# sachaMorin/dino

Measured on AMD Instinct MI355X. Metric: frames/sec (480x480, ViT-S/8) DINOSeg inference, higher is better.
Workload: dtype fp16 (linears, Q.K^T; P.V bf16; fp32 accumulate); 1 GPU; DINOSeg predict path: ViT-S/8 x12 blocks + MLP head, 480x480 uint8 frames, batch 32/GPU, frames resident in HBM; blocks=12, batch_per_gpu=32, global_batch=32, resolution=480, precision=fp16, streams=2, parallelism=dp1 (independent replicas, no data-path collective)

## Files before the change

dino_amd/csrc/kernels.h:

```cpp
#pragma once
#include <hip/hip_runtime.h>
#include <stdint.h>

struct dinoseg_augment_frame;

namespace dseg {

typedef uint16_t bf16_t;

enum GemmEpilogue {
    EPI_PLAIN = 0,
    EPI_RESID = 1,
    EPI_GELU = 2,
    EPI_RELU = 3,
    EPI_QKV = 4,
    EPI_PATCH = 5,
    EPI_BF16 = 6,
    EPI_ATOMIC = 7,
    EPI_DGELU = 8,
    EPI_DRELU = 9,
};

struct GemmParams {
    const bf16_t* A; long a_plane; int lda;
    const bf16_t* W; long w_plane;
    int M, N, K;
    int n_off;
    int n_valid;
    int dbg;
    int planes;
    int fmt;
    int epi;
    const float* bias;
    float* out_f32; int ldo_f32;
    bf16_t* out_bf16; long out_plane; int ldo;
    bf16_t* q; bf16_t* k; bf16_t* v; long qkv_plane;
    int ntok, npad, heads, dmodel; float qscale;
    const float* pos; int n_patches;
    const float* resid;
    bf16_t* aux_out;
    const bf16_t* aux_in; long aux_plane;
    int v_bf16;
    int dispatch_rows;
    int ksplit;
    long split_stride;
    const float* ln_x; float ln_eps;
};
int launch_gemm(const GemmParams& p, hipStream_t s);
int launch_gemm_small(const GemmParams& p, hipStream_t s);
bool gemm_big_supported(const GemmParams& p);
int launch_gemm_big(const GemmParams& p, hipStream_t s);

bool gemm_rs_supported(const GemmParams& p);
int launch_pack_rs(const float* W, int N, int K, int kind, bf16_t* dst, hipStream_t s, int fmt);
int launch_pack_rs_ln(const float* W, const float* gamma, const float* beta, const float* bias, int N, int K, bf16_t* dst_w, float* dst_bias,
                      hipStream_t s, int fmt);
int launch_gemm_rs(const GemmParams& p, hipStream_t s);

struct LnGemmParams {
    const float* X; int ldx;
    const float* gamma; const float* beta; float eps;
    const bf16_t* W; long w_plane;
    const float* bias;
    int M, N;
    int epi;
    bf16_t* out_bf16; long out_plane; int ldo;
    bf16_t* q; bf16_t* k; bf16_t* v; long qkv_plane; int ntok, npad, heads, dmodel; float qscale;
    bf16_t* a_out; long a_plane;
    bf16_t* aux_out; long aux_plane;
    int dbg;
    int fmt;
};
bool gemm_ln_supported(int K, int N, int planes, int epi, int dmodel);
long gemm_ln_slab_elems(int N, int K, int planes);
int launch_pack_slabs(const float* src, int N, int K, int planes, bf16_t* dst, hipStream_t s, int fmt = 0);
int launch_gemm_ln(const LnGemmParams& p, int K, int planes, hipStream_t s);

struct MlpFusedParams {
    float* X; int ldx;
    const float* gamma; const float* beta; float eps;
    const bf16_t* Wp;
    const float* b1; const float* b2;
    int M;
    int* queue;
    int n_long, sleep_max;
    const bf16_t* ctx;
    const bf16_t* Wproj;
    const float* bproj;
    const bf16_t* Wqkv;
    const float* bqkv; const float* gamma1; const float* beta1;
    bf16_t* q; bf16_t* k; bf16_t* v;
    int ntok, npad, heads; float qscale;
    int fmt;
};
long mlp_fused_qkv_pack_elems(int D);
int launch_pack_qkv(const float* W, int D, bf16_t* dst, hipStream_t s, int fmt = 0);
long mlp_fused_proj_pack_elems(int D);
int launch_pack_proj(const float* W, int D, bf16_t* dst, hipStream_t s, int fmt = 0);
bool mlp_fused_supported(int D, int F, int planes);
long mlp_fused_pack_elems(int D, int F);
int launch_pack_mlp(const float* W1, const float* W2, int D, int F, bf16_t* dst, hipStream_t s, int fmt = 0);
int launch_mlp_fused2(const MlpFusedParams& p, hipStream_t s);

struct MlpFused3Params {
    float* X;
    float eps;
    const bf16_t* Wp;
    const float* b2;
    int M;
    const bf16_t* ctx; long ctx_plane;
    const float* bproj;
    int fmt;
    bf16_t* q; bf16_t* k; bf16_t* v; long qkv_plane;
    int ntok, npad, heads; float qscale;
    int v_bf16;
};
struct MlpFused3Weights {
    const float* Wproj; const float* W1; const float* b1; const float* W2;
    const float* gamma2; const float* beta2;
    const float* Wqkv_next; const float* bqkv_next; const float* gamma1_next; const float* beta1_next;
};
bool mlp_fused3_supported(int D, int F, int planes);
long mlp_fused3_pack_elems(int D, int F);
int launch_pack_mlp3(const MlpFused3Weights& w, int D, int F, bf16_t* dst, hipStream_t s, int fmt);
int launch_mlp_fused3(const MlpFused3Params& p, hipStream_t s);
bool mlp_fused4_supported(int D, int F, int planes);
long mlp_fused4_pack_elems(int D, int F);
int launch_pack_mlp4(const MlpFused3Weights& w, int D, int F, bf16_t* dst, hipStream_t s, int fmt);
int launch_mlp_fused4(const MlpFused3Params& p, hipStream_t s);

struct Options {
    int gemm_ln = 1;
    int gemm_big = 1;
    int gemm_dbg = 0;
    int attn_dbg = 0;
    int mlp_fused = 1;
    int mlp_fused_min_rows = 12000;
    int mlp_fused3_min_rows = 10000;
    int mlp_stagger = 0;
    int mlp_grid = 0;
    int qkv_fused = 0;
    int mlp_fused4 = 0;
    int qkv_fused4 = 1;
    int qkv_fused3 = 1;
    int gemm_rs = 3;
    int gemm_rs_min_rows = 24000;
    int gemm_rs_ln = 1;
    int proj_fused = 1;
    int streams = 2;
    int split_min = 8;
    int route_ab = 0;
    int fp16_patch_planes = 1;
    int op_v_bf16 = 0;
    int op_fmt = 0;
    int deterministic = 0;
    int train_streams = 2;
    int splitk_tiles = 512;
    int attn_variant = 11 | 1024 | 65536;
};
Options& options();

struct AttnParams {
    const bf16_t* q; const bf16_t* k; const bf16_t* v; long qkv_plane;
    bf16_t* ctx; long ctx_plane;
    float* lse;
    int B, heads, ntok, npad, planes;
    int dbg;
    int shared_gpu;
// ... 169 lines not shown
```

dino_amd/csrc/mlp_fused2.hip:

```cpp
#include <stdio.h>

#include <vector>

#include "mlp_common.h"

namespace dseg {

namespace mf2 {
using namespace mfc;
constexpr int NP = 4, BM = NP * 32, THREADS = 2 * NP * 64;
constexpr int W1_OFF = 0, W2_OFF = 3 * W_TILE;
constexpr int P_OFF = W2_OFF + 2 * W_TILE;
constexpr int B1_OFF = P_OFF + NP * 2 * 2048;
constexpr int B2_OFF = B1_OFF + F * 4;
constexpr int G_OFF = B2_OFF + D * 4, BE_OFF = G_OFF + D * 4;
constexpr int BP_OFF = BE_OFF + D * 4;
constexpr int G1_OFF = BP_OFF + D * 4, BE1_OFF = G1_OFF + D * 4;
constexpr int BQ_OFF = BE1_OFF + D * 4;
constexpr int NQT = 3 * D / 32;
constexpr int LDS_BYTES = BQ_OFF + 3 * D * 4;
static_assert(LDS_BYTES <= 160 * 1024, "LDS budget");
constexpr int NPT = D / 32;
constexpr int CTX_OFF = W2_OFF, CTX_SLOT = BM * 64;
static_assert(6 * CTX_SLOT == 2 * W_TILE, "ctx ring = W2 ring");
constexpr int H_OFF = W2_OFF + W_TILE;
static_assert(H_OFF + NP * 8192 <= B1_OFF, "hand-off windows");
#ifndef MF2_RA
#define MF2_RA 4
#endif
constexpr int RA = MF2_RA, NFR = RA + 1;
}

#ifndef MF2_ABL
#define MF2_ABL 0
#endif

#ifndef MF2_NT
#define MF2_NT 0
#endif
template <class T>
__device__ __forceinline__ T mf2_ld(const T* p) {
    if (MF2_NT & 1) return __builtin_nontemporal_load(p);
    return *p;
}
template <class T>
__device__ __forceinline__ void mf2_st(T* p, const T& v) {
    if (MF2_NT & 2) __builtin_nontemporal_store(v, p);
    else *p = v;
}

#ifndef MF2_STAMP
#define MF2_STAMP 0
#endif
#define MF2_ST(role, item_k, idx)                                                                                         \
    do {                                                                                                                  \
        if (MF2_STAMP && (tid & 63) == 0 && (item_k) < 4) {                                                               \
            __builtin_amdgcn_sched_barrier(0);                                                                            \
            unsigned long long* d = reinterpret_cast<unsigned long long*>(p.queue) +                                      \
                                    ((((long)blockIdx.x * 2 + (role)) * 4 + (item_k)) * 16 + (idx)) * 2;                  \
            d[0] = __builtin_amdgcn_s_memrealtime();                                                                      \
            d[1] = __builtin_amdgcn_s_memtime();                                                                          \
            __builtin_amdgcn_sched_barrier(0);                                                                            \
        }                                                                                                                 \
    } while (0)

template <int FMT, class PieceFn>
__device__ __forceinline__ void mf2_proj_tile(f32x16 (&acc)[mfc::NDB], uint32_t a_w, uint32_t ap0, uint32_t ap1, PieceFn&& piece) {
    using namespace mf2;
    bf16x8 p0, p1, fr[NFR];
    mf_rd<0>(p0, ap0);
    mf_rd<0>(p1, ap1);
    auto issue_read = [&](auto g_tag) __attribute__((always_inline)) {
        constexpr int G = decltype(g_tag)::value;
        if constexpr (G < 12) mf_rd<(2 * G) * 1024>(fr[G % NFR], a_w);
        else mf_rd<(2 * (G - 12) + 1) * 1024>(fr[G % NFR], a_w);
    };
    mf_for(std::make_integer_sequence<int, RA>{}, issue_read);
    mf_for(std::make_integer_sequence<int, 24>{}, [&](auto g_tag) __attribute__((always_inline)) {
        constexpr int G = decltype(g_tag)::value;
        if constexpr (G + RA < 24) issue_read(std::integral_constant<int, G + RA>{});
        mf_wait<(23 - G < RA ? 23 - G : RA)>();
        acc[G % 12] = mfma32f<FMT>(fr[G % NFR], G < 12 ? p0 : p1, acc[G % 12]);
        __builtin_amdgcn_sched_barrier(0);
        if constexpr ((G & 1) == 0) piece(std::integral_constant<int, G / 2>{});
        __builtin_amdgcn_sched_barrier(0);
    });
}

template <bool PROJ, bool QKV, int FMT>
__global__ __launch_bounds__(mf2::THREADS, 2) void mlp_fused2_kernel(MlpFusedParams p) {
    static_assert(PROJ || !QKV, "the qkv tail needs the hand-off machinery of the projection build");
    using namespace mf2;
    extern __shared__ __attribute__((aligned(16))) char smem[];
    const int tid = threadIdx.x;
    const int wave = __builtin_amdgcn_readfirstlane(tid >> 6);
    const int pair = wave & 3;
    const bool is_b = wave >= 4;
    const int M = p.M;
    const int nitems = (M + BM - 1) / BM;
    if ((int)blockIdx.x >= nitems) return;

    {
        float* const sB1w = reinterpret_cast<float*>(smem + B1_OFF);
        for (int i = tid; i < F / 4; i += THREADS) reinterpret_cast<f32x4*>(sB1w)[i] = reinterpret_cast<const f32x4*>(p.b1)[i];
        for (int i = tid; i < 3 * D / 4; i += THREADS) {
            const int which = i / (D / 4), j = i - which * (D / 4);
            const float* src = which == 0 ? p.b2 : (which == 1 ? p.gamma : p.beta);
            if (PROJ && which == 0) src = p.bproj;
            reinterpret_cast<f32x4*>(smem + B2_OFF + which * D * 4)[j] = reinterpret_cast<const f32x4*>(src)[j];
        }
        if (PROJ)
            for (int i = tid; i < D / 4; i += THREADS) reinterpret_cast<f32x4*>(smem + BP_OFF)[i] = reinterpret_cast<const f32x4*>(p.b2)[i];
        if (QKV) {
            for (int i = tid; i < 2 * D / 4; i += THREADS)
                reinterpret_cast<f32x4*>(smem + G1_OFF)[i] = reinterpret_cast<const f32x4*>(i < D / 4 ? p.gamma1 : p.beta1)[i < D / 4 ? i : i - D / 4];
            for (int i = tid; i < 3 * D / 4; i += THREADS) reinterpret_cast<f32x4*>(smem + BQ_OFF)[i] = reinterpret_cast<const f32x4*>(p.bqkv)[i];
        }
    }
    if (p.sleep_max > 0 && (int)blockIdx.x >= p.n_long) {
        const int n_short = (int)gridDim.x - p.n_long;
        const int reps = (int)(((long)p.sleep_max * ((int)blockIdx.x - p.n_long + 1)) / n_short);
        for (int i = 0; i < reps; ++i) __builtin_amdgcn_s_sleep(127);
    }
    const uint32_t lds_base = (uint32_t)(size_t)(__attribute__((address_space(3))) char*)smem;
    const float* const sB1 = reinterpret_cast<const float*>(smem + B1_OFF);
    const float* const sB2 = reinterpret_cast<const float*>(smem + B2_OFF);
    const float* const sG = reinterpret_cast<const float*>(smem + G_OFF);
    const float* const sBe = reinterpret_cast<const float*>(smem + BE_OFF);
    auto uniform64 = [](uint64_t v) __attribute__((always_inline)) -> uint64_t {
        return (uint64_t)(uint32_t)__builtin_amdgcn_readfirstlane((uint32_t)v) |
               ((uint64_t)(uint32_t)__builtin_amdgcn_readfirstlane((uint32_t)(v >> 32)) << 32);
    };
// ... 79 lines not shown
            };
            if (item == (int)blockIdx.x) load_rows(xrow);
            if (wave == 4) MF2_ST(1, item_k, 1);

            auto step_b = [&](int s, auto kind_tag) __attribute__((always_inline)) {
                constexpr int KIND = decltype(kind_tag)::value;
                __builtin_amdgcn_s_barrier();
                const int v1 = s + 3;
                const bool has_w2 = PROJ ? (s >= 1 && s <= NT - 1) : s <= NT - 1, has_w1 = v1 != NT;
                const int t1 = v1 < NT ? v1 : v1 - (NT + 1);
                const bool nxt = PROJ && v1 > NT;
                uint64_t gsb[4];
                uint32_t gld[4];
                {
                    const uint32_t so2 = (uint32_t)s * TILE_BYTES + W_TILE + frag0;
                    const uint32_t so1 = (nxt ? (uint32_t)t1 * W_TILE : (uint32_t)t1 * TILE_BYTES) + frag0;
                    const uint32_t d2 = lds_base + W2_OFF + (uint32_t)(s & 1) * W_TILE + frag0;
                    const uint32_t d1 = lds_base + W1_OFF + (uint32_t)(t1 % 3) * W_TILE + frag0;
                    const uint64_t w1src = nxt ? (QKV ? wq : wpj) : wp;
                    gsb[0] = uniform64(wp + so2);
                    gsb[1] = uniform64(wp + so2 + 4096);
                    gsb[2] = uniform64(w1src + so1);
                    gsb[3] = uniform64(w1src + so1 + 4096);
                    gld[0] = __builtin_amdgcn_readfirstlane(d2);
                    gld[1] = __builtin_amdgcn_readfirstlane(d2 + 4096);
                    gld[2] = __builtin_amdgcn_readfirstlane(d1);
                    gld[3] = __builtin_amdgcn_readfirstlane(d1 + 4096);
                }
                const bool ctx_pre = PROJ && s == NT && item + (int)gridDim.x < nitems;
                uint32_t cvn[2] = {0u, 0u};
                if (ctx_pre) {
#pragma unroll
                    for (int j = 0; j < 2; ++j) {
                        const uint32_t rin = (uint32_t)(2 * pair + j) * 16 + (lane_i >> 2);
                        int rg = (item + (int)gridDim.x) * BM + (int)rin;
                        rg = rg < M ? rg : M - 1;
                        cvn[j] = (uint32_t)rg * (D * 2) + (((lane_i & 3) ^ ((rin >> 2) & 3)) << 4);
                    }
                }
                auto piece = [&](auto j_tag) __attribute__((always_inline)) {
                    constexpr int J = decltype(j_tag)::value;
                    if (MF2_ABL & 2) return;
                    if constexpr (PROJ && J < 6) {
                        if (ctx_pre) {
                            constexpr int T = J >> 1, JJ = J & 1;
                            mf_dma1<0>(cvn[JJ], uniform64(ctxb + T * 64),
                                       __builtin_amdgcn_readfirstlane(lds_base + CTX_OFF + T * CTX_SLOT + (uint32_t)(2 * pair + JJ) * 1024));
                        }
                    }
                    if (J < 6 ? !has_w2 : !has_w1) return;
                    constexpr int Q = J % 6, G4 = (J / 6) * 2 + (Q >= 4 ? 1 : 0), OFF = (Q & 3) * 1024;
                    mf_dma1<OFF>(lane16_i, gsb[G4], gld[G4]);
                };
                if constexpr (KIND == 0) {
                    mf_for(std::make_integer_sequence<int, 12>{}, piece);
                    asm volatile("s_waitcnt vmcnt(6)" ::: "memory");
                } else {
                    const uint32_t a2 = frag_rd_i + W2_OFF + (uint32_t)((s - 1) & 1) * W_TILE;
                    const uint32_t ap = p_rd_i + (uint32_t)((s - 1) & 1) * 2048;
                    bf16x8 p0, p1, fr[NFR];
                    mf_rd<0>(p0, ap);
                    mf_rd<1024>(p1, ap);
                    auto issue_read = [&](auto g_tag) __attribute__((always_inline)) {
                        constexpr int G = decltype(g_tag)::value;
                        if (MF2_ABL & 16) return;
                        if constexpr (G < 12) mf_rd<(2 * G) * 1024>(fr[G % NFR], a2);
                        else mf_rd<(2 * (G - 12) + 1) * 1024>(fr[G % NFR], a2);
                    };
                    mf_for(std::make_integer_sequence<int, RA>{}, issue_read);
                    mf_for(std::make_integer_sequence<int, 24>{}, [&](auto g_tag) __attribute__((always_inline)) {
                        constexpr int G = decltype(g_tag)::value;
                        if constexpr (G + RA < 24) issue_read(std::integral_constant<int, G + RA>{});
                        if (MF2_ABL & 16) fr[G % NFR] = p0;
                        else mf_wait<(23 - G < RA ? 23 - G : RA)>();
                        if (!(MF2_ABL & 8)) o[G % 12] = mfma32f<FMT>(fr[G % NFR], G < 12 ? p0 : p1, o[G % 12]);
                        __builtin_amdgcn_sched_barrier(0);
                        if constexpr ((G & 1) == 0) piece(std::integral_constant<int, G / 2>{});
                        __builtin_amdgcn_sched_barrier(0);
                    });
                    if (s == NT - 3) asm volatile("s_waitcnt vmcnt(0)" ::: "memory");
                    else asm volatile("s_waitcnt vmcnt(6)" ::: "memory");
                }
            };
            auto ln_handoff = [&](const float* sGam, const float* sBet) __attribute__((always_inline)) {
                float sum = 0.f;
#pragma unroll
                for (int db = 0; db < NDB; ++db)
#pragma unroll
                    for (int h = 0; h < 2; ++h)
                        sum += ((o[db][8 * h] + o[db][8 * h + 1]) + (o[db][8 * h + 2] + o[db][8 * h + 3])) +
                               ((o[db][8 * h + 4] + o[db][8 * h + 5]) + (o[db][8 * h + 6] + o[db][8 * h + 7]));
                sum += __shfl_xor(sum, 32);
                const float mean = sum * (1.0f / D);
                float qv = 0.f;
#pragma unroll
                for (int db = 0; db < NDB; ++db)
#pragma unroll
                    for (int q4 = 0; q4 < 4; ++q4) {
                        __builtin_amdgcn_sched_barrier(0);
                        float part = 0.f;
#pragma unroll
                        for (int e = 0; e < 4; ++e) {
                            const float dlt = o[db][4 * q4 + e] - mean;
                            part = fmaf(dlt, dlt, part);
                        }
                        qv += part;
                    }
                qv += __shfl_xor(qv, 32);
                const float rstd = 1.0f / sqrtf(qv * (1.0f / D) + p.eps);
                float mean_n = mean;
                asm volatile("" : "+v"(mean_n));
                char* const hw = smem + H_OFF + pair * 8192 + lane16_i;
#pragma unroll
                for (int r = 0; r < 3; ++r) {
                    if (r > 0) __builtin_amdgcn_s_barrier();
#pragma unroll
                    for (int kk = 0; kk < 8; ++kk) {
                        __builtin_amdgcn_sched_barrier(0);
                        const int k = r * 8 + kk;
                        const float* gp = sGam + k * 16 + lh_i * 8;
                        const float* bp = sBet + k * 16 + lh_i * 8;
                        const f32x4 g0 = *reinterpret_cast<const f32x4*>(gp), g1 = *reinterpret_cast<const f32x4*>(gp + 4);
                        const f32x4 e0 = *reinterpret_cast<const f32x4*>(bp), e1 = *reinterpret_cast<const f32x4*>(bp + 4);
                        float y[8];
#pragma unroll
                        for (int e = 0; e < 4; ++e) {
                            y[e] = (o[k >> 1][(k & 1) * 8 + e] - mean_n) * rstd * g0[e] + e0[e];
                            y[4 + e] = (o[k >> 1][(k & 1) * 8 + 4 + e] - mean_n) * rstd * g1[e] + e1[e];
                        }
                        uint4 u;
                        u.x = pack2<FMT>(y[0], y[1]);
                        u.y = pack2<FMT>(y[2], y[3]);
                        u.z = pack2<FMT>(y[4], y[5]);
                        u.w = pack2<FMT>(y[6], y[7]);
                        *reinterpret_cast<uint4*>(hw + kk * 1024) = u;
                    }
                    asm volatile("s_waitcnt lgkmcnt(0)" ::: "memory");
                    if (r < 2) __builtin_amdgcn_s_barrier();
                }
            };

            if constexpr (PROJ) {
                uint32_t cv[2];
#pragma unroll
                for (int j = 0; j < 2; ++j) {
                    const uint32_t rin = (uint32_t)(2 * pair + j) * 16 + (lane_i >> 2);
                    int rg = item * BM + (int)rin;
                    rg = rg < M ? rg : M - 1;
                    cv[j] = (uint32_t)rg * (D * 2) + (((lane_i & 3) ^ ((rin >> 2) & 3)) << 4);
                }
                const uint32_t cp0 = ctx_frag_addr(lr_i, lh_i);
#pragma unroll 1
                for (int kt = 0; kt < NPT; ++kt) {
                    __builtin_amdgcn_s_barrier();
                    const bool issue = kt >= 1 && kt + 2 < NPT;
                    const int t = kt + 2;
                    const uint32_t so = (uint32_t)t * W_TILE + frag0;
                    const uint32_t d = lds_base + W1_OFF + (uint32_t)(t % 3) * W_TILE + frag0;
                    const uint32_t dc = lds_base + CTX_OFF + (uint32_t)(t % 6) * CTX_SLOT + (uint32_t)(2 * pair) * 1024;
                    const uint64_t gb0 = uniform64(wpj + so), gb1 = uniform64(wpj + so + 4096), cb = uniform64(ctxb + (uint32_t)t * 64);
                    const uint32_t gl0 = __builtin_amdgcn_readfirstlane(d), gl1 = __builtin_amdgcn_readfirstlane(d + 4096);
                    const uint32_t cl0 = __builtin_amdgcn_readfirstlane(dc), cl1 = __builtin_amdgcn_readfirstlane(dc + 1024);
                    auto piece = [&](auto j_tag) __attribute__((always_inline)) {
                        constexpr int J = decltype(j_tag)::value;
                        if ((MF2_ABL & 2) || !issue) return;
                        if constexpr (J < 4) mf_dma1<J * 1024>(lane16_i, gb0, gl0);
                        else if constexpr (J < 6) mf_dma1<(J - 4) * 1024>(lane16_i, gb1, gl1);
                        else if constexpr (J == 6) mf_dma1<0>(cv[0], cb, cl0);
                        else if constexpr (J == 7) mf_dma1<0>(cv[1], cb, cl1);
                    };
                    const uint32_t cs = (uint32_t)(kt % 6) * CTX_SLOT;
                    mf2_proj_tile<FMT>(o, frag_rd_i + W1_OFF + (uint32_t)(kt % 3) * W_TILE, cp0 + cs, (cp0 ^ 32u) + cs, piece);
                    if (issue) asm volatile("s_waitcnt vmcnt(8)" ::: "memory");
                    else asm volatile("s_waitcnt vmcnt(0)" ::: "memory");
                }
                if (wave == 4) MF2_ST(1, item_k, 9);
                __builtin_amdgcn_s_barrier();
                if (!(MF2_ABL & 2)) {
#pragma unroll
                    for (int t = 0; t < 4; ++t) {
                        const uint64_t sb = uniform64(wp + (t < 3 ? (uint32_t)t * TILE_BYTES : (uint32_t)W_TILE) + frag0);
                        const uint32_t ld = __builtin_amdgcn_readfirstlane(lds_base + (t < 3 ? W1_OFF + t * W_TILE : W2_OFF) + frag0);
                        mf_dma4(lane16_i, sb, ld);
                        mf_dma1<0>(lane16_i, sb + 4096, ld + 4096);
                        mf_dma1<1024>(lane16_i, sb + 4096, ld + 4096);
                    }
                }
                ln_handoff(sG, sBe);
                asm volatile("s_waitcnt vmcnt(0)" ::: "memory");
                if (wave == 4) MF2_ST(1, item_k, 10);
                __builtin_amdgcn_s_barrier();
                if (wave == 4) MF2_ST(1, item_k, 11);
            }
            step_b(0, std::integral_constant<int, 0>{});
            if (wave == 4) MF2_ST(1, item_k, 2);
#pragma unroll 1
            for (int s = 1; s <= NT; ++s) {
                step_b(s, std::integral_constant<int, 1>{});
                if (wave == 4 && s == 1) MF2_ST(1, item_k, 3);
                if (wave == 4 && s == 24) MF2_ST(1, item_k, 4);
                if (wave == 4 && s == 47) MF2_ST(1, item_k, 5);
            }
            if (wave == 4) MF2_ST(1, item_k, 6);

            if constexpr (QKV) {
                const bool has_next = item + (int)gridDim.x < nitems;
                {
                    const float* fp = reinterpret_cast<const float*>(smem + BP_OFF) + lh_i * 8;
#pragma unroll
                    for (int k = 0; k < NKS; ++k) {
                        const f32x4 c0 = *reinterpret_cast<const f32x4*>(fp + k * 16), c1 = *reinterpret_cast<const f32x4*>(fp + k * 16 + 4);
#pragma unroll
                        for (int e = 0; e < 4; ++e) {
                            o[k >> 1][(k & 1) * 8 + e] += c0[e];
                            o[k >> 1][(k & 1) * 8 + 4 + e] += c1[e];
                        }
                    }
                }
                __builtin_amdgcn_s_barrier();
                ln_handoff(reinterpret_cast<const float*>(smem + G1_OFF), reinterpret_cast<const float*>(smem + BE1_OFF));
                asm volatile("s_waitcnt vmcnt(0)" ::: "memory");
                __builtin_amdgcn_s_barrier();
                const int fr_ = row_c / p.ntok, tok_ = row_c - fr_ * p.ntok;
                const long qkv_row = ((long)fr_ * p.heads * p.npad + tok_) * 64 + lh_i * 8;
                const float* const nxr = p.X + (long)((row + BM * (int)gridDim.x) < M ? row + BM * (int)gridDim.x : M - 1) * D + lh_i * 8;
                mf_for(std::make_integer_sequence<int, NQT + 1>{}, [&](auto t_tag) __attribute__((always_inline)) {
                    constexpr int T = decltype(t_tag)::value;
                    __builtin_amdgcn_s_barrier();
                    if constexpr (T >= 1) {
                        constexpr int TT = T - 1, WHICH = TT / NDB, HB = TT % NDB;
                        const char* pr = smem + P_OFF + pair * 4096 + lane16_i + (TT & 1) * 2048;
                        const uint4 u0 = *reinterpret_cast<const uint4*>(pr), u1 = *reinterpret_cast<const uint4*>(pr + 1024);
                        bf16_t* dst = (WHICH == 0 ? p.q : (WHICH == 1 ? p.k : p.v)) + qkv_row + (long)(HB >> 1) * p.npad * 64 + (HB & 1) * 32;
                        if (row < M) {
                            *reinterpret_cast<uint4*>(dst) = u0;
                            *reinterpret_cast<uint4*>(dst + 16) = u1;
                        }
                    }
                    if constexpr (T >= 1 && T <= NKS) {
                        constexpr int k = T - 1;
                        if (row < M) {
                            f32x4 a, b;
#pragma unroll
                            for (int e = 0; e < 4; ++e) {
                                a[e] = o[k >> 1][(k & 1) * 8 + e];
                                b[e] = o[k >> 1][(k & 1) * 8 + 4 + e];
                            }
                            mf2_st(reinterpret_cast<f32x4*>(xrow + k * 16), a);
                            mf2_st(reinterpret_cast<f32x4*>(xrow + k * 16 + 4), b);
                        }
                    }
                    if constexpr (T > NKS) {
                        if (has_next) {
                            load_rows_k(nxr, std::integral_constant<int, 2 * (T - NKS - 1)>{});
                            load_rows_k(nxr, std::integral_constant<int, 2 * (T - NKS - 1) + 1>{});
                        }
                    }
                });
                static_assert(NQT + 1 - NKS - 1 == NKS / 2, "row loads fill the steps behind the row stores");
                if (has_next && !(MF2_ABL & 2)) {
#pragma unroll
                    for (int t = 0; t < 3; ++t) {
                        const uint64_t sb = uniform64(wpj + (uint32_t)t * W_TILE + frag0);
                        const uint32_t ld = __builtin_amdgcn_readfirstlane(lds_base + W1_OFF + t * W_TILE + frag0);
                        mf_dma4(lane16_i, sb, ld);
                        mf_dma1<0>(lane16_i, sb + 4096, ld + 4096);
                        mf_dma1<1024>(lane16_i, sb + 4096, ld + 4096);
                    }
                }
                asm volatile("s_waitcnt vmcnt(0)" ::: "memory");
                continue;
            }
            if (MF2_ABL & 32) {
#pragma unroll
                for (int db = 0; db < NDB; ++db) asm volatile("" ::"v"(o[db]));
            } else if (row < M) {
#pragma unroll
                for (int k = 0; k < NKS; ++k) {
                    f32x4 a, b;
#pragma unroll
                    for (int e = 0; e < 4; ++e) {
                        a[e] = o[k >> 1][(k & 1) * 8 + e];
                        b[e] = o[k >> 1][(k & 1) * 8 + 4 + e];
                    }
                    if constexpr (PROJ) {
                        const float* fp = reinterpret_cast<const float*>(smem + BP_OFF) + k * 16 + lh_i * 8;
                        a += *reinterpret_cast<const f32x4*>(fp);
                        b += *reinterpret_cast<const f32x4*>(fp + 4);
                    }
                    mf2_st(reinterpret_cast<f32x4*>(xrow + k * 16), a);
                    mf2_st(reinterpret_cast<f32x4*>(xrow + k * 16 + 4), b);
                }
            }
            if (wave == 4) MF2_ST(1, item_k, 7);
            if (item + (int)gridDim.x < nitems) {
                const int nrow = row + BM * (int)gridDim.x;
                load_rows(p.X + (long)(nrow < M ? nrow : M - 1) * D + lh_i * 8);
            }
            if (wave == 4) MF2_ST(1, item_k, 8);
        }
        asm volatile("s_waitcnt vmcnt(0)" ::: "memory");
        return;
    }
// ... 70 lines not shown
        const int row = item * BM + pair * 32 + lr;
        const int row_c = row < M ? row : M - 1;
        const float* const xrow = p.X + (long)row_c * D + lh * 8;
        f32x4 x[2 * NKS];
#pragma unroll
        for (int k = 0; k < NKS; ++k) {
            if (MF2_ABL & 32) {
                x[2 * k] = f32x4{1.f, 2.f, (float)k, (float)lane_p};
                x[2 * k + 1] = x[2 * k];
            } else {
                x[2 * k] = mf2_ld(reinterpret_cast<const f32x4*>(xrow + k * 16));
                x[2 * k + 1] = mf2_ld(reinterpret_cast<const f32x4*>(xrow + k * 16 + 4));
            }
        }
        layernorm(x, lh);
        return s_zero(lane_p, sB1);
    };
#define MF2_GELU2 0
    constexpr int GELU_LAST = MF2_GELU2 ? 8 : 10;
    float ex[16], ea[16], eb[16], ec[16];
    uint32_t pd[8];
    auto gelu_op = [&](auto n_tag, auto i_tag, const f32x16& s) __attribute__((always_inline)) {
        constexpr int N = decltype(n_tag)::value, I = decltype(i_tag)::value;
        if constexpr (I == 0) ex[N] = s[N];
        if (MF2_ABL & 1) {
            if constexpr (I == GELU_LAST && (N & 1)) pd[N >> 1] = pack2<FMT>(ex[N - 1], ex[N]);
            return;
        }
        if constexpr (MF2_GELU2) {
            if constexpr (I == 1) eb[N] = ex[N] * ex[N];
            if constexpr (I == 2) ec[N] = fmaf(-1.00125610e-1f, eb[N], -2.30876530f);
            if constexpr (I == 3) ec[N] = ec[N] * ex[N];
            if constexpr (I == 4) ec[N] = __builtin_amdgcn_exp2f(ec[N]);
            if constexpr (I == 5) ec[N] = 1.0f + ec[N];
            if constexpr (I == 6) ec[N] = __builtin_amdgcn_rcpf(ec[N]);
            if constexpr (I == 7) ex[N] = ex[N] * ec[N];
        } else {
            if constexpr (I == 1) ea[N] = __builtin_amdgcn_fmed3f(ex[N], -8.0f, 8.0f);
            if constexpr (I == 2) eb[N] = ea[N] * ea[N];
            if constexpr (I == 3) ec[N] = fmaf(1.01537542e-3f, eb[N], -1.06782573e-1f);
            if constexpr (I == 4) ec[N] = fmaf(ec[N], eb[N], -2.30111381f);
            if constexpr (I == 5) ec[N] = ec[N] * ea[N];
            if constexpr (I == 6) ec[N] = __builtin_amdgcn_exp2f(ec[N]);
            if constexpr (I == 7) ec[N] = 1.0f + ec[N];
            if constexpr (I == 8) ec[N] = __builtin_amdgcn_rcpf(ec[N]);
            if constexpr (I == 9) ex[N] = ex[N] * ec[N];
        }
        if constexpr (I == GELU_LAST && (N & 1)) pd[N >> 1] = pack2<FMT>(ex[N - 1], ex[N]);
    };
    auto valu_slot = [&](auto g_tag, const f32x16& s) __attribute__((always_inline)) {
        constexpr int G = decltype(g_tag)::value;
        mf_for(std::make_integer_sequence<int, 16>{}, [&](auto n_tag) __attribute__((always_inline)) {
            constexpr int N = decltype(n_tag)::value;
            constexpr int SG = (14 * N) / 15;
            if constexpr (G >= SG && G - SG <= GELU_LAST) gelu_op(n_tag, std::integral_constant<int, G - SG>{}, s);
        });
    };

    if (wave == 0) MF2_ST(0, 0, 15);
    if constexpr (!PROJ) sa = prologue(blockIdx.x);
    int item_k = 0;
    for (int item = blockIdx.x; item < nitems; item += gridDim.x, ++item_k) {
        if (wave == 0) MF2_ST(0, item_k, 0);
        uint32_t zero = 0;
        asm volatile("" : "+v"(zero));
        const uint32_t lane_i = __builtin_amdgcn_mbcnt_hi(~0u, __builtin_amdgcn_mbcnt_lo(~0u, zero));
        const uint32_t lane16_i = lane_i * 16, lh_i = lane_i >> 5;
        const uint32_t frag_rd_i = lds_base + lane16_i;
        char* const p_wr = smem + P_OFF + pair * 4096 + lane16_i;
        const float* const b1_lane_p = sB1 + attn::sigma23((int)(lane_i & 31));
        constexpr uint32_t ONE = FMT == FMT_FP16 ? 0x3C00u : 0x3F80u;
        const uint4 ones_u = {lh_i == 0 ? (ONE << 16 | ONE) : 0u, lh_i == 0 ? ONE : 0u, 0u, 0u};
        auto receive_xn = [&]() __attribute__((always_inline)) {
            const char* const hr = smem + H_OFF + pair * 8192 + lane16_i;
#pragma unroll
            for (int r = 0; r < 3; ++r) {
                __builtin_amdgcn_s_barrier();
#pragma unroll
                for (int kk = 0; kk < 8; ++kk) xn[r * 8 + kk] = lds_frag(hr + kk * 1024);
                asm volatile("s_waitcnt lgkmcnt(0)" ::: "memory");
                if (r < 2) __builtin_amdgcn_s_barrier();
            }
        };
        if constexpr (PROJ) {
#pragma unroll 1
            for (int kt = 0; kt <= NPT; ++kt) __builtin_amdgcn_s_barrier();
            receive_xn();
            sa = s_zero((int)lane_i, sB1);
            if (wave == 0) MF2_ST(0, item_k, 10);
        }

        auto step_a = [&](f32x16& s_cur, f32x16& s_nxt, int s, auto last_tag) __attribute__((always_inline)) {
            constexpr bool LAST = decltype(last_tag)::value;
            bf16x8 bias_frag;
            if (!LAST) {
                const float bj = b1_lane_p[(s + 1) * HT];
                const uint32_t hi = pack2<FMT>(bj, 0.f);
                const float r1f = bj - lo_to_f32<FMT>(hi);
                const uint32_t mid = pack2<FMT>(r1f, 0.f);
                const uint32_t lo = pack2<FMT>(r1f - lo_to_f32<FMT>(mid), 0.f);
                const uint4 fu = {lh_i == 0 ? ((hi & 0xFFFFu) | (mid << 16)) : 0u, lh_i == 0 ? (lo & 0xFFFFu) : 0u, 0u, 0u};
                bias_frag = __builtin_bit_cast(bf16x8, fu);
            }
            __builtin_amdgcn_sched_barrier(0);
            __builtin_amdgcn_s_barrier();
            if constexpr (!LAST) {
                const uint32_t a1 = frag_rd_i + W1_OFF + (uint32_t)((s + 1) % 3) * W_TILE;
                bf16x8 fr[NFR];
                auto issue_read = [&](auto g_tag) __attribute__((always_inline)) {
                    constexpr int G = decltype(g_tag)::value;
                    if (MF2_ABL & 16) return;
                    mf_rd<G * 1024>(fr[G % NFR], a1);
                };
                mf_for(std::make_integer_sequence<int, RA>{}, issue_read);
                {
                    f32x16 z;
#pragma unroll
                    for (int r = 0; r < 16; ++r) z[r] = 0.f;
                    s_nxt = mfma32f<FMT>(bias_frag, __builtin_bit_cast(bf16x8, ones_u), z);
                }
                __builtin_amdgcn_sched_barrier(0);
                mf_for(std::make_integer_sequence<int, 24>{}, [&](auto g_tag) __attribute__((always_inline)) {
                    constexpr int G = decltype(g_tag)::value;
                    if constexpr (G + RA < 24) issue_read(std::integral_constant<int, G + RA>{});
                    if (MF2_ABL & 16) fr[G % NFR] = xn[(G + 1) % NKS];
                    else mf_wait<(23 - G < RA ? 23 - G : RA)>();
                    if (!(MF2_ABL & 4)) s_nxt = mfma32f<FMT>(fr[G % NFR], xn[G], s_nxt);
                    __builtin_amdgcn_sched_barrier(0);
                    valu_slot(g_tag, s_cur);
                    __builtin_amdgcn_sched_barrier(0);
                });
                valu_slot(std::integral_constant<int, 24>{}, s_cur);
            } else {
                mf_for(std::make_integer_sequence<int, 25>{}, [&](auto g_tag) __attribute__((always_inline)) { valu_slot(g_tag, s_cur); });
            }
            const uint4 u0 = {pd[0], pd[1], pd[2], pd[3]}, u1 = {pd[4], pd[5], pd[6], pd[7]};
            *reinterpret_cast<uint4*>(p_wr + (s & 1) * 2048) = u0;
            *reinterpret_cast<uint4*>(p_wr + (s & 1) * 2048 + 1024) = u1;
            asm volatile("s_waitcnt lgkmcnt(0)" ::: "memory");
            __builtin_amdgcn_sched_barrier(0);
        };
#pragma unroll 1
        for (int s = 0; s < NT - 2; s += 2) {
            step_a(sa, sb, s, std::false_type{});
            if (wave == 0 && s == 0) MF2_ST(0, item_k, 1);
            step_a(sb, sa, s + 1, std::false_type{});
            if (wave == 0 && s == 0) MF2_ST(0, item_k, 2);
            if (wave == 0 && s == 22) MF2_ST(0, item_k, 3);
        }
        if (wave == 0) MF2_ST(0, item_k, 4);
        step_a(sa, sb, NT - 2, std::false_type{});
        step_a(sb, sa, NT - 1, std::true_type{});
        if (wave == 0) MF2_ST(0, item_k, 5);
        __builtin_amdgcn_s_barrier();
        if (wave == 0) MF2_ST(0, item_k, 6);
        if constexpr (QKV) {
            __builtin_amdgcn_s_barrier();
            receive_xn();
            const float* const sBq = reinterpret_cast<const float*>(smem + BQ_OFF);
            const float* const bq_lane_p = sBq + attn::sigma23((int)(lane_i & 31));
            const uint32_t frag0 = (uint32_t)pair * 6 * 1024;
            sa = s_zero((int)lane_i, sBq);
            auto step_q = [&](f32x16& s_cur, f32x16& s_nxt, int t, auto last_tag) __attribute__((always_inline)) {
                constexpr bool LAST = decltype(last_tag)::value;
                bf16x8 bias_frag;
                if (!LAST) {
                    const float bj = bq_lane_p[(t + 1) * 32];
                    const uint32_t hi = pack2<FMT>(bj, 0.f);
                    const float r1f = bj - lo_to_f32<FMT>(hi);
                    const uint32_t mid = pack2<FMT>(r1f, 0.f);
                    const uint32_t lo = pack2<FMT>(r1f - lo_to_f32<FMT>(mid), 0.f);
// ... 114 lines not shown
    for (int idx = blockIdx.x * blockDim.x + threadIdx.x; idx < total; idx += gridDim.x * blockDim.x) {
        int t = idx;
        const int e = t & 7; t >>= 3;
        const int lane = t & 63; t >>= 6;
        const int frag = t % NKS, kt = t / NKS;
        const int i = attn::sigma23(lane & 31), h = lane >> 5, db = frag >> 1, s2 = frag & 1;
        dst[idx] = pack1(W[(long)(db * 32 + i) * D + kt * 32 + s2 * 16 + h * 8 + e], fmt);
    }
}
__global__ __launch_bounds__(256) void pack_qkv_kernel(const float* __restrict__ W, bf16_t* __restrict__ dst, int fmt) {
    using namespace mf2;
    const int total = NQT * NKS * 512;
    for (int idx = blockIdx.x * blockDim.x + threadIdx.x; idx < total; idx += gridDim.x * blockDim.x) {
        int t = idx;
        const int e = t & 7; t >>= 3;
        const int lane = t & 63; t >>= 6;
        const int frag = t % NKS, tile = t / NKS;
        const int i = attn::sigma23(lane & 31), h = lane >> 5;
        dst[idx] = pack1(W[(long)(tile * 32 + i) * D + frag * 16 + h * 8 + e], fmt);
    }
}
long mlp_fused_qkv_pack_elems(int Dm) { return Dm == mf2::D ? (long)mf2::NQT * mf2::W_TILE / 2 : 0; }
int launch_pack_qkv(const float* W, int Dm, bf16_t* dst, hipStream_t s, int fmt) {
    if (Dm != mf2::D) {
        dinoseg_set_error("pack_qkv: unsupported width %d", Dm);
        return -1;
    }
    hipLaunchKernelGGL(pack_qkv_kernel, dim3(432), dim3(256), 0, s, W, dst, fmt);
    DSEG_CHECK_HIP(hipGetLastError());
    return 0;
}

long mlp_fused_proj_pack_elems(int Dm) { return Dm == mf2::D ? (long)mf2::NPT * mf2::W_TILE / 2 : 0; }
int launch_pack_proj(const float* W, int Dm, bf16_t* dst, hipStream_t s, int fmt) {
    if (Dm != mf2::D) {
        dinoseg_set_error("pack_proj: unsupported width %d", Dm);
        return -1;
    }
    hipLaunchKernelGGL(pack_proj_kernel, dim3(144), dim3(256), 0, s, W, dst, fmt);
    DSEG_CHECK_HIP(hipGetLastError());
    return 0;
}

template <int FMT>
static int launch_mlp_fused2_fmt(const MlpFusedParams& p, hipStream_t s);

int launch_mlp_fused2(const MlpFusedParams& p, hipStream_t s) {
    return p.fmt == FMT_FP16 ? launch_mlp_fused2_fmt<FMT_FP16>(p, s) : launch_mlp_fused2_fmt<FMT_BF16>(p, s);
}

template <int FMT>
static int launch_mlp_fused2_fmt(const MlpFusedParams& p, hipStream_t s) {
    static PerDeviceOnce once;
    if (once.first()) {
        DSEG_CHECK_HIP(hipFuncSetAttribute(reinterpret_cast<const void*>(&mlp_fused2_kernel<false, false, FMT>),
                                           hipFuncAttributeMaxDynamicSharedMemorySize, mf2::LDS_BYTES));
        DSEG_CHECK_HIP(hipFuncSetAttribute(reinterpret_cast<const void*>(&mlp_fused2_kernel<true, false, FMT>),
                                           hipFuncAttributeMaxDynamicSharedMemorySize, mf2::LDS_BYTES));
        DSEG_CHECK_HIP(hipFuncSetAttribute(reinterpret_cast<const void*>(&mlp_fused2_kernel<true, true, FMT>),
                                           hipFuncAttributeMaxDynamicSharedMemorySize, mf2::LDS_BYTES));
        once.mark();
    }
    if (p.M <= 0 || p.ldx != mf2::D) {
        dinoseg_set_error("mlp_fused2: bad shape M=%d ldx=%d", p.M, p.ldx);
        return -1;
    }
    const int ncu = device_cu_count();
    if (ncu <= 0) return -2;
    const int nitems = (p.M + mf2::BM - 1) / mf2::BM;
    int grid;
    if (options().mlp_stagger > 0) {
        grid = nitems < ncu ? nitems : ncu;
    } else if (options().mlp_grid > 0) {
        grid = options().mlp_grid < ncu ? options().mlp_grid : ncu;
        if (grid > nitems) grid = nitems;
    } else {
        const int rounds = (nitems + ncu - 1) / ncu;
        grid = (nitems + rounds - 1) / rounds;
    }
    MlpFusedParams q = p;
    q.queue = nullptr;
    q.n_long = nitems % grid;
    q.sleep_max = q.n_long > 0 && nitems > grid ? options().mlp_stagger : 0;
#if MF2_STAMP
    static unsigned long long* sbuf = nullptr;
    const size_t sbytes = (size_t)grid * 2 * 4 * 16 * 2 * 8;
    if (!sbuf) DSEG_CHECK_HIP(hipMalloc(reinterpret_cast<void**>(&sbuf), 256 * 2 * 4 * 16 * 2 * 8));
    DSEG_CHECK_HIP(hipMemsetAsync(sbuf, 0, sbytes, s));
    q.queue = reinterpret_cast<int*>(sbuf);
#endif
    if (p.ctx) {
        if (!p.Wproj || !p.bproj) {
            dinoseg_set_error("mlp_fused2: ctx without the packed projection weight / bias");
            return -1;
        }
        if (p.Wqkv) {
            if (!p.bqkv || !p.gamma1 || !p.beta1 || !p.q || !p.k || !p.v || p.ntok <= 0 || p.npad < p.ntok || p.heads * 64 != mf2::D) {
                dinoseg_set_error("mlp_fused2: incomplete qkv tail (bias / norm1 / q / k / v / geometry)");
                return -1;
            }
            hipLaunchKernelGGL((mlp_fused2_kernel<true, true, FMT>), dim3(grid), dim3(mf2::THREADS), mf2::LDS_BYTES, s, q);
        } else {
            hipLaunchKernelGGL((mlp_fused2_kernel<true, false, FMT>), dim3(grid), dim3(mf2::THREADS), mf2::LDS_BYTES, s, q);
        }
    } else {
        if (p.Wqkv) {
            dinoseg_set_error("mlp_fused2: the qkv tail needs the projection in the same launch (ctx)");
            return -1;
        }
        hipLaunchKernelGGL((mlp_fused2_kernel<false, false, FMT>), dim3(grid), dim3(mf2::THREADS), mf2::LDS_BYTES, s, q);
    }
    DSEG_CHECK_HIP(hipGetLastError());
#if MF2_STAMP
    {
        static int calls = 0;
        if (++calls == 20) {
            DSEG_CHECK_HIP(hipStreamSynchronize(s));
            std::vector<unsigned long long> h(sbytes / 8);
            DSEG_CHECK_HIP(hipMemcpy(h.data(), sbuf, sbytes, hipMemcpyDeviceToHost));
            for (int role = 0; role < 2; ++role)
                for (int k = 0; k < 4; ++k) {
                    fprintf(stderr, "role %c item %d:", role ? 'B' : 'A', k);
                    for (int i = 0; i < 16; ++i) {
                        double sum = 0, sumc = 0;
                        int n = 0;
                        for (int b = 0; b < grid; ++b) {
                            const unsigned long long* d = &h[((((size_t)b * 2 + role) * 4 + k) * 16) * 2];
                            const unsigned long long* d0 = &h[((((size_t)b * 2 + 1) * 4 + 0) * 16) * 2];
                            if (d[2 * i] == 0 || d0[0] == 0) continue;
                            sum += (double)(d[2 * i] - d0[0]) * 0.01;
                            sumc += (double)(d[2 * i + 1] - d0[1]);
                            ++n;
                        }
                        if (n) fprintf(stderr, " [%d] %.1fus/%.0fkc", i, sum / n, sumc / n / 1e3);
                    }
                    fprintf(stderr, "\n");
                }
        }
    }
#endif
    return 0;
}

}
```

Baseline: 2603 frames/s.

## Swap projection DMA/MFMA roles between wave pairs and overlap first hidden step with LN handoff

Reassigns work inside the fused attention-projection/MLP kernel. The consumer-side waves now issue the projection weight and context DMAs, and the producer waves run the projection MFMAs directly from LDS without prefetching. The first MLP hidden-layer step is folded into receiving the normalized activations, so MFMA work starts while rounds arrive instead of after all three. The LN handoff also relaxes a vmcnt wait to let loads stay in flight. The old placement stays available through a flag, at the cost of extra code paths and a more delicate barrier/waitcnt protocol.

```diff
diff --git a/dino_amd/csrc/kernels.h b/dino_amd/csrc/kernels.h
--- a/dino_amd/csrc/kernels.h
+++ b/dino_amd/csrc/kernels.h
@@ -84,6 +84,7 @@
     int M;
     int* queue;
     int n_long, sleep_max;
+    int old_place;
     const bf16_t* ctx;
     const bf16_t* Wproj;
     const float* bproj;
diff --git a/dino_amd/csrc/mlp_fused2.hip b/dino_amd/csrc/mlp_fused2.hip
--- a/dino_amd/csrc/mlp_fused2.hip
+++ b/dino_amd/csrc/mlp_fused2.hip
@@ -48,6 +48,10 @@
     if (MF2_NT & 2) __builtin_nontemporal_store(v, p);
     else *p = v;
 }
+
+#ifndef MF2_PLACE
+#define MF2_PLACE 0
+#endif
 
 #ifndef MF2_STAMP
 #define MF2_STAMP 0
@@ -293,7 +297,7 @@
                     else asm volatile("s_waitcnt vmcnt(6)" ::: "memory");
                 }
             };
-            auto ln_handoff = [&](const float* sGam, const float* sBet) __attribute__((always_inline)) {
+            auto ln_handoff = [&](const float* sGam, const float* sBet, bool early) __attribute__((always_inline)) {
                 float sum = 0.f;
 #pragma unroll
                 for (int db = 0; db < NDB; ++db)
@@ -347,6 +351,7 @@
                         *reinterpret_cast<uint4*>(hw + kk * 1024) = u;
                     }
                     asm volatile("s_waitcnt lgkmcnt(0)" ::: "memory");
+                    if (r == 0 && early) asm volatile("s_waitcnt vmcnt(18)" ::: "memory");
                     if (r < 2) __builtin_amdgcn_s_barrier();
                 }
             };
@@ -361,8 +366,17 @@
                     cv[j] = (uint32_t)rg * (D * 2) + (((lane_i & 3) ^ ((rin >> 2) & 3)) << 4);
                 }
                 const uint32_t cp0 = ctx_frag_addr(lr_i, lh_i);
+                if (!(p.old_place & 1)) {
 #pragma unroll 1
-                for (int kt = 0; kt < NPT; ++kt) {
+                    for (int kt = 0; kt < NPT; ++kt) {
+                        __builtin_amdgcn_s_barrier();
+                        const uint32_t cs = (uint32_t)(kt % 6) * CTX_SLOT;
+                        mf2_proj_tile<FMT>(o, frag_rd_i + W1_OFF + (uint32_t)(kt % 3) * W_TILE, cp0 + cs, (cp0 ^ 32u) + cs, [](auto) {});
+                        asm volatile("s_waitcnt vmcnt(0)" ::: "memory");
+                    }
+                }
+#pragma unroll 1
+                for (int kt = (p.old_place & 1) ? 0 : NPT; kt < NPT; ++kt) {
                     __builtin_amdgcn_s_barrier();
                     const bool issue = kt >= 1 && kt + 2 < NPT;
                     const int t = kt + 2;
@@ -397,7 +411,7 @@
                         mf_dma1<1024>(lane16_i, sb + 4096, ld + 4096);
                     }
                 }
-                ln_handoff(sG, sBe);
+                ln_handoff(sG, sBe, !(p.old_place & 2));
                 asm volatile("s_waitcnt vmcnt(0)" ::: "memory");
                 if (wave == 4) MF2_ST(1, item_k, 10);
                 __builtin_amdgcn_s_barrier();
@@ -429,7 +443,7 @@
                     }
                 }
                 __builtin_amdgcn_s_barrier();
-                ln_handoff(reinterpret_cast<const float*>(smem + G1_OFF), reinterpret_cast<const float*>(smem + BE1_OFF));
+                ln_handoff(reinterpret_cast<const float*>(smem + G1_OFF), reinterpret_cast<const float*>(smem + BE1_OFF), false);
                 asm volatile("s_waitcnt vmcnt(0)" ::: "memory");
                 __builtin_amdgcn_s_barrier();
                 const int fr_ = row_c / p.ntok, tok_ = row_c - fr_ * p.ntok;
@@ -666,11 +680,95 @@
                 if (r < 2) __builtin_amdgcn_s_barrier();
             }
         };
+        auto receive_xn_s0 = [&]() __attribute__((always_inline)) {
+            const char* const hr = smem + H_OFF + pair * 8192 + lane16_i;
+            f32x16 s;
+            {
+                const float* bp = sB1 + lh_i * 8;
+                const f32x4 c0 = *reinterpret_cast<const f32x4*>(bp), c1 = *reinterpret_cast<const f32x4*>(bp + 4);
+                const f32x4 c2 = *reinterpret_cast<const f32x4*>(bp + 16), c3 = *reinterpret_cast<const f32x4*>(bp + 20);
+#pragma unroll
+                for (int e = 0; e < 4; ++e) {
+                    s[e] = c0[e];
+                    s[4 + e] = c1[e];
+                    s[8 + e] = c2[e];
+                    s[12 + e] = c3[e];
+                }
+            }
+            static_assert(RA <= 8, "the read-ahead stays inside a round's eight k-steps");
+            const uint32_t a1 = frag_rd_i + W1_OFF;
+            mf_for(std::make_integer_sequence<int, 3>{}, [&](auto r_tag) __attribute__((always_inline)) {
+                constexpr int R = decltype(r_tag)::value;
+                __builtin_amdgcn_s_barrier();
+#pragma unroll
+                for (int kk = 0; kk < 8; ++kk) xn[R * 8 + kk] = lds_frag(hr + kk * 1024);
+                asm volatile("s_waitcnt lgkmcnt(0)" ::: "memory");
+                if constexpr (R < 2) __builtin_amdgcn_s_barrier();
+                __builtin_amdgcn_sched_barrier(0);
+                bf16x8 fr[NFR];
+                auto issue_read = [&](auto g_tag) __attribute__((always_inline)) {
+                    constexpr int G = decltype(g_tag)::value;
+                    mf_rd<G * 1024>(fr[G % NFR], a1);
+                };
+                mf_for(std::make_integer_sequence<int, RA>{}, [&](auto g_tag) __attribute__((always_inline)) {
+                    issue_read(std::integral_constant<int, R * 8 + decltype(g_tag)::value>{});
+                });
+                mf_for(std::make_integer_sequence<int, 8>{}, [&](auto g_tag) __attribute__((always_inline)) {
+                    constexpr int GG = decltype(g_tag)::value, G = R * 8 + GG;
+                    if constexpr (GG + RA < 8) issue_read(std::integral_constant<int, G + RA>{});
+                    mf_wait<(7 - GG < RA ? 7 - GG : RA)>();
+                    s = mfma32f<FMT>(fr[G % NFR], xn[G], s);
+                    __builtin_amdgcn_sched_barrier(0);
+                });
+            });
+            return s;
+        };
         if constexpr (PROJ) {
+            if (p.old_place & 1) {
 #pragma unroll 1
-            for (int kt = 0; kt <= NPT; ++kt) __builtin_amdgcn_s_barrier();
-            receive_xn();
-            sa = s_zero((int)lane_i, sB1);
+                for (int kt = 0; kt <= NPT; ++kt) __builtin_amdgcn_s_barrier();
+            } else {
+                const uint32_t frag0 = (uint32_t)pair * 6 * 1024;
+                uint32_t cv[2];
+#pragma unroll
+                for (int j = 0; j < 2; ++j) {
+                    const uint32_t rin = (uint32_t)(2 * pair + j) * 16 + (lane_i >> 2);
+                    int rg = item * BM + (int)rin;
+                    rg = rg < M ? rg : M - 1;
+                    cv[j] = (uint32_t)rg * (D * 2) + (((lane_i & 3) ^ ((rin >> 2) & 3)) << 4);
+                }
+#pragma unroll 1
+                for (int kt = 0; kt < NPT; ++kt) {
+                    __builtin_amdgcn_s_barrier();
+                    const bool issue = kt >= 1 && kt + 2 < NPT;
+                    const int t = kt + 2;
+                    const uint32_t so = (uint32_t)t * W_TILE + frag0;
+                    const uint32_t d = lds_base + W1_OFF + (uint32_t)(t % 3) * W_TILE + frag0;
+                    const uint32_t dc = lds_base + CTX_OFF + (uint32_t)(t % 6) * CTX_SLOT + (uint32_t)(2 * pair) * 1024;
+                    const uint64_t gb0 = uniform64(wpj + so), gb1 = uniform64(wpj + so + 4096), cb = uniform64(ctxb + (uint32_t)t * 64);
+                    const uint32_t gl0 = __builtin_amdgcn_readfirstlane(d), gl1 = __builtin_amdgcn_readfirstlane(d + 4096);
+                    const uint32_t cl0 = __builtin_amdgcn_readfirstlane(dc), cl1 = __builtin_amdgcn_readfirstlane(dc + 1024);
+                    if (issue && !(MF2_ABL & 2)) {
+                        mf_dma1<0>(lane16_i, gb0, gl0);
+                        mf_dma1<1024>(lane16_i, gb0, gl0);
+                        mf_dma1<2048>(lane16_i, gb0, gl0);
+                        mf_dma1<3072>(lane16_i, gb0, gl0);
+                        mf_dma1<0>(lane16_i, gb1, gl1);
+                        mf_dma1<1024>(lane16_i, gb1, gl1);
+                        mf_dma1<0>(cv[0], cb, cl0);
+                        mf_dma1<0>(cv[1], cb, cl1);
+                    }
+                    if (issue) asm volatile("s_waitcnt vmcnt(8)" ::: "memory");
+                    else asm volatile("s_waitcnt vmcnt(0)" ::: "memory");
+                }
+                __builtin_amdgcn_s_barrier();
+            }
+            if (p.old_place & 2) {
+                receive_xn();
+                sa = s_zero((int)lane_i, sB1);
+            } else {
+                sa = receive_xn_s0();
+            }
             if (wave == 0) MF2_ST(0, item_k, 10);
         }
 
@@ -951,6 +1049,7 @@
     q.queue = nullptr;
     q.n_long = nitems % grid;
     q.sleep_max = q.n_long > 0 && nitems > grid ? options().mlp_stagger : 0;
+    q.old_place = (options().route_ab & 8) ? 3 : MF2_PLACE;
 #if MF2_STAMP
     static unsigned long long* sbuf = nullptr;
     const size_t sbytes = (size_t)grid * 2 * 4 * 16 * 2 * 8;
```

Measured after the change: 2614 frames/s, median of 6. No clear change (+0.4%).
